# pdeljanov/Symphonia

Hardware: NVIDIA H100
Metric: decoded audio-seconds/sec (44.1kHz stereo) (higher is better)
Workload: dtype f32

## Files before the change

symphonia_b200/csrc/mp3_kernel.cu:

```cuda
#include <cuda_runtime.h>

#include <cstdint>
#include <cstdlib>

#include "../../include/symgpu.h"
#include "mp3_kernel.h"
#include "tables.h"

namespace symgpu {

struct Mp3Const {
    float imdct_win[4][36];
    float half_cos12[6][6];
    float dct_iv_scale[18];
    float sdct18_scale[9];
    float sdct9_d[7];
    float lee16[16], lee8[8], lee4[4], lee2[2], lee1;
    float is_mpeg1[7][2];
    float is_mpeg2[2][32][2];
    float cs[8], ca[8];
    uint8_t pre_emphasis[24];
    uint8_t mixed_switch[12];
    uint8_t n_edges[9][3];
};
__constant__ Mp3Const c_mp3;

cudaError_t mp3_upload_const(const Mp3Tables& t, cudaStream_t stream) {
    static Mp3Const h;
    memcpy(h.imdct_win, t.imdct_win, sizeof h.imdct_win);
    memcpy(h.half_cos12, t.half_cos12, sizeof h.half_cos12);
    memcpy(h.dct_iv_scale, t.dct_iv_scale, sizeof h.dct_iv_scale);
    memcpy(h.sdct18_scale, t.sdct18_scale, sizeof h.sdct18_scale);
    memcpy(h.sdct9_d, t.sdct9_d, sizeof h.sdct9_d);
    memcpy(h.lee16, t.lee16, sizeof h.lee16);
    memcpy(h.lee8, t.lee8, sizeof h.lee8);
    memcpy(h.lee4, t.lee4, sizeof h.lee4);
    memcpy(h.lee2, t.lee2, sizeof h.lee2);
    h.lee1 = t.lee1;
    memcpy(h.is_mpeg1, t.is_mpeg1, sizeof h.is_mpeg1);
    memcpy(h.is_mpeg2, t.is_mpeg2, sizeof h.is_mpeg2);
    memcpy(h.cs, t.cs, sizeof h.cs);
    memcpy(h.ca, t.ca, sizeof h.ca);
    memcpy(h.pre_emphasis, t.pre_emphasis, sizeof h.pre_emphasis);
    memset(h.mixed_switch, 0, sizeof h.mixed_switch);
    memcpy(h.mixed_switch, t.mixed_switch, 9);
    memcpy(h.n_edges, t.n_edges, sizeof h.n_edges);
    cudaError_t e = cudaMemcpyToSymbolAsync(c_mp3, &h, sizeof h, 0, cudaMemcpyHostToDevice, stream);
    if (e != cudaSuccess) return e;
    return cudaStreamSynchronize(stream);
}

namespace {

constexpr int kPitch = 33;
constexpr float kFrac1Sqrt2 = 0.707106781186547524400844362104849039f;

struct WarpScratch {
    symgpu_mp3_gc gc[2];
    float scale[2][40];
    float2 sratio[40];
    uint8_t smode[40];
    uint8_t nz[40];
    int next_region;
    Mp3StreamState* st_out;
};

__device__ __forceinline__ int kind_of(const symgpu_mp3_gc& g) {
    if (g.block_type != SYMGPU_MP3_SHORT) return kKindLong;
    return (g.flags & SYMGPU_MP3_F_MIXED) ? kKindMixed : kKindShort;
}

__device__ __forceinline__ void sdct9(const float (&x)[9], float (&y)[9]) {
    const float a01 = x[3] + x[5], a02 = x[3] - x[5], a03 = x[6] + x[2], a04 = x[6] - x[2];
    const float a05 = x[1] + x[7], a06 = x[1] - x[7], a07 = x[8] + x[0], a08 = x[8] - x[0];
    const float a09 = x[4] + a05, a10 = a01 + a03, a11 = a10 + a07, a12 = a03 - a07;
    const float a13 = a01 - a07, a14 = a01 - a03, a15 = a02 - a04, a16 = a15 + a08;
    const float a17 = a04 + a08, a18 = a02 - a08, a19 = a02 + a04, a20 = 2.0f * x[4] - a05;
    const float m1 = c_mp3.sdct9_d[0] * a06, m2 = c_mp3.sdct9_d[1] * a12, m3 = c_mp3.sdct9_d[2] * a13;
    const float m4 = c_mp3.sdct9_d[3] * a14, m5 = c_mp3.sdct9_d[0] * a16, m6 = c_mp3.sdct9_d[4] * a17;
    const float m7 = c_mp3.sdct9_d[5] * a18, m8 = c_mp3.sdct9_d[6] * a19;
    const float a21 = a20 + m2, a22 = a20 - m2, a23 = a20 + m3, a24 = m1 + m6, a25 = m1 - m6, a26 = m1 + m7;
    y[0] = a09 + a11;
    y[1] = m8 - a26;
    y[2] = m4 - a21;
    y[3] = m5;
    y[4] = a22 - m3;
    y[5] = a25 - m7;
    y[6] = a11 - 2.0f * a09;
    y[7] = a24 + m8;
    y[8] = a23 + m4;
}

__device__ __forceinline__ void dct_iv_18(const float (&x)[18], float (&y)[18]) {
    float s[18];
#pragma unroll
    for (int i = 0; i < 18; ++i) s[i] = c_mp3.dct_iv_scale[i] * x[i];
    float even[9], odd[9], ye[9], yo[9];
#pragma unroll
    for (int i = 0; i < 9; ++i) even[i] = s[i] + s[17 - i];
    sdct9(even, ye);
#pragma unroll
    for (int i = 0; i < 9; ++i) odd[i] = c_mp3.sdct18_scale[i] * (s[i] - s[17 - i]);
    sdct9(odd, yo);
#pragma unroll
    for (int j = 1; j < 9; ++j) yo[j] = yo[j] - yo[j - 1];
#pragma unroll
    for (int j = 0; j < 9; ++j) {
        y[2 * j] = ye[j];
        y[2 * j + 1] = yo[j];
    }
    y[0] = y[0] * 0.5f;
#pragma unroll
    for (int i = 1; i < 18; ++i) y[i] = (y[i] * 0.5f) - y[i - 1];
}

__device__ __forceinline__ void imdct36(const float (&x)[18], const float* __restrict__ win,
                                        float (&first)[18], float (&second)[18]) {
// ... 20 lines not shown
        for (int i = 0; i < 3; ++i) {
            const float yl = (x[w] * c_mp3.half_cos12[i][0]) + (x[3 + w] * c_mp3.half_cos12[i][1]) +
                             (x[6 + w] * c_mp3.half_cos12[i][2]) + (x[9 + w] * c_mp3.half_cos12[i][3]) +
                             (x[12 + w] * c_mp3.half_cos12[i][4]) + (x[15 + w] * c_mp3.half_cos12[i][5]);
            const float yr = (x[w] * c_mp3.half_cos12[i + 3][0]) + (x[3 + w] * c_mp3.half_cos12[i + 3][1]) +
                             (x[6 + w] * c_mp3.half_cos12[i + 3][2]) + (x[9 + w] * c_mp3.half_cos12[i + 3][3]) +
                             (x[12 + w] * c_mp3.half_cos12[i + 3][4]) + (x[15 + w] * c_mp3.half_cos12[i + 3][5]);
            tmp[6 + 6 * w + 2 - i] += -yl * win[2 - i];
            tmp[6 + 6 * w + i + 3] += yl * win[i + 3];
            tmp[6 + 6 * w + i + 6] += yr * win[i + 6];
            tmp[6 + 6 * w + 11 - i] += yr * win[11 - i];
        }
    }
#pragma unroll
    for (int i = 0; i < 18; ++i) {
        first[i] = tmp[i];
        second[i] = tmp[i + 18];
    }
}

template <int N> struct LeeCoef;
template <> struct LeeCoef<16> { static __device__ __forceinline__ float at(int i) { return c_mp3.lee16[i]; } };
template <> struct LeeCoef<8> { static __device__ __forceinline__ float at(int i) { return c_mp3.lee8[i]; } };
template <> struct LeeCoef<4> { static __device__ __forceinline__ float at(int i) { return c_mp3.lee4[i]; } };
template <> struct LeeCoef<2> { static __device__ __forceinline__ float at(int i) { return c_mp3.lee2[i]; } };

template <int N>
__device__ __forceinline__ void lee_dct(const float (&x)[N], float (&y)[N]) {
    if constexpr (N == 2) {
        y[0] = x[0] + x[1];
        y[1] = (x[0] - x[1]) * c_mp3.lee1;
    } else {
        constexpr int H = N / 2;
        float lo[H], hi[H], lo_t[H], hi_t[H];
#pragma unroll
        for (int i = 0; i < H; ++i) {
            lo[i] = x[i] + x[N - 1 - i];
            hi[i] = (x[i] - x[N - 1 - i]) * LeeCoef<H>::at(i);
        }
        lee_dct<H>(lo, lo_t);
        lee_dct<H>(hi, hi_t);
#pragma unroll
        for (int i = 0; i < H - 1; ++i) {
            y[2 * i] = lo_t[i];
            y[2 * i + 1] = hi_t[i] + hi_t[i + 1];
        }
        y[N - 2] = lo_t[H - 1];
        y[N - 1] = hi_t[H - 1];
    }
}

__device__ __forceinline__ float finv(float v, int sb, int t) { return ((sb & t) & 1) ? -v : v; }

}

namespace {

__device__ __forceinline__ uint32_t smem_u32(const void* p) { return (uint32_t)__cvta_generic_to_shared(p); }
__device__ __forceinline__ void mbar_init(uint64_t* bar, uint32_t count) {
    asm volatile("mbarrier.init.shared::cta.b64 [%0], %1;" ::"r"(smem_u32(bar)), "r"(count) : "memory");
}
__device__ __forceinline__ void mbar_expect_tx(uint64_t* bar, uint32_t bytes) {
    asm volatile("mbarrier.arrive.expect_tx.shared::cta.b64 _, [%0], %1;" ::"r"(smem_u32(bar)), "r"(bytes) : "memory");
}
__device__ __forceinline__ void mbar_wait(uint64_t* bar, uint32_t parity) {
    asm volatile(
        "{\n"
        ".reg .pred p;\n"
        "WAIT_%=:\n"
        "mbarrier.try_wait.parity.shared::cta.b64 p, [%0], %1;\n"
        "@p bra DONE_%=;\n"
        "bra WAIT_%=;\n"
        "DONE_%=:\n"
        "}\n" ::"r"(smem_u32(bar)),
        "r"(parity)
        : "memory");
}
__device__ __forceinline__ void tma_bulk_g2s(void* dst_smem, const void* src_gmem, uint32_t bytes, uint64_t* bar) {
    asm volatile("cp.async.bulk.shared::cluster.global.mbarrier::complete_tx::bytes [%0], [%1], %2, [%3];" ::"r"(
                     smem_u32(dst_smem)),
                 "l"(src_gmem), "r"(bytes), "r"(smem_u32(bar))
                 : "memory");
}

__device__ __forceinline__ float2 lds64(uint32_t addr) {
    float2 v;
    asm volatile("ld.shared.v2.f32 {%0, %1}, [%2];" : "=f"(v.x), "=f"(v.y) : "r"(addr));
    return v;
}


__device__ __forceinline__ float2 pk_mul(float2 a, float s) { return make_float2(__fmul_rn(a.x, s), __fmul_rn(a.y, s)); }
__device__ __forceinline__ float2 pk_add(float2 a, float2 b) { return make_float2(__fadd_rn(a.x, b.x), __fadd_rn(a.y, b.y)); }

template <bool TWO_JUMPS = false>
__device__ __forceinline__ void window_phase(const float* xt, int row0, int begin, int end, int lane,
                                             const float* __restrict__ synth_d, float* __restrict__ pcm, int slot_seq0,
                                             int slots_per_frame, bool stereo) {
    const int col_lo = lane < 16 ? 16 + lane : (lane == 16 ? 32 : 48 - lane);
    const int col_hi = lane <= 16 ? 16 - lane : lane - 16;
    float dlo[8], dhi[8];
#pragma unroll
    for (int j = 0; j < 8; ++j) {
        const float a0 = __ldg(synth_d + 64 * j + lane);
        dlo[j] = lane > 16 ? -a0 : a0;
        dhi[j] = -__ldg(synth_d + 64 * j + 32 + lane);
    }
    if (begin >= end) return;
    constexpr uint32_t kRowBytes = kPitch * 8;
    uint32_t a_lo = smem_u32(xt) + (uint32_t)((row0 + begin - 15) * kPitch + col_lo) * 8u;
    uint32_t a_hi = smem_u32(xt) + (uint32_t)((row0 + begin - 15) * kPitch + col_hi) * 8u;
    float2 wl[16], wh[16];
#pragma unroll
    for (int m = 0; m < 15; ++m) {
        wl[(m + 1) & 15] = lds64(a_lo + m * kRowBytes);
        wh[(m + 1) & 15] = lds64(a_hi + m * kRowBytes);
    }
    a_lo += 15 * kRowBytes;
    a_hi += 15 * kRowBytes;
    const int off1 = stereo ? 1152 : 0;
    const int frame_jump = SYMGPU_MP3_FRAME_FLOATS - slots_per_frame * 32;
    for (int base = begin; base < end; base += 16) {
        const int seq = slot_seq0 + base;
        const int frame = seq / slots_per_frame, sif = seq - frame * slots_per_frame;
        float* out0 = pcm + (size_t)frame * SYMGPU_MP3_FRAME_FLOATS + sif * 32 + lane;
        float* out1 = out0 + frame_jump;
        const int kj = slots_per_frame - sif;
        const int cnt = end - base;
#pragma unroll
        for (int u = 0; u < 16; ++u) {
            if (u < cnt) {
                wl[u] = lds64(a_lo + u * kRowBytes);
                wh[u] = lds64(a_hi + u * kRowBytes);
                float2 acc = make_float2(0.0f, 0.0f);
#pragma unroll
                for (int j = 0; j < 8; ++j) {
                    acc = pk_add(pk_mul(wl[(u - 2 * j) & 15], dlo[j]), acc);
                    acc = pk_add(pk_mul(wh[(u - 2 * j - 1) & 15], dhi[j]), acc);
                }
                float* o = (u < kj ? out0 : out1) + u * 32;
                if (TWO_JUMPS && u >= kj + slots_per_frame) o += frame_jump;
                o[off1] = acc.y;
                o[0] = acc.x;
            }
        }
        a_lo += 16 * kRowBytes;
        a_hi += 16 * kRowBytes;
    }
}

template <int T, int NW>
struct Mp3Smem {
    static constexpr int kRows = 18 * kMp3GroupRegions;
    float xt[kRows * kPitch * 2];
    alignas(16) float spec[NW][2 * 576];
    alignas(16) symgpu_mp3_gc units[NW][2];
    WarpScratch ws[NW];
    alignas(16) Mp3StreamState carry;
    alignas(16) Mp3Tile seg_stage[2][kMp3GroupTiles];
    uint32_t gen_stage[2][kMp3GroupTiles];
    int nseg_stage[2];
    alignas(8) uint64_t bar;
    bool is_last;
};

}

template <int T, int NW, bool MULTI>
__global__ void __launch_bounds__(NW * 32, NW <= 8 ? 2 : 1) mp3_synth_kernel(Mp3Args a) {
    static_assert(NW >= T, "one warp per granule job (a tile with a halo holds NW - 2 granules)");
    extern __shared__ __align__(16) unsigned char smem_raw[];
    using Smem = Mp3Smem<T, NW>;
    Smem& sm = *reinterpret_cast<Smem*>(smem_raw);
    float* xt = sm.xt;

    const int lane = threadIdx.x & 31;
    const int warp = threadIdx.x >> 5;
    const Mp3Tables* __restrict__ tab = a.tab;
    const int n_tiles = a.n_tiles;

    auto issue_prefetch = [&](int ti, int parity) {
        int nseg = 0, jobs = 0;
        for (;;) {
            const Mp3Tile t = a.tiles[ti + nseg];
            sm.seg_stage[parity][nseg] = t;
            sm.gen_stage[parity][nseg] = a.gen[t.stream];
            jobs += t.n_granules + ((t.flags & (kTileLoadState | kTileCarryIn)) ? 0 : 2);
            ++nseg;
            if (!MULTI || (t.flags & kTileGroupEnd) || nseg == kMp3GroupTiles) break;
        }
        sm.nseg_stage[parity] = nseg;
        mbar_expect_tx(&sm.bar, (uint32_t)jobs * (4608u + 128u));
        int slot0 = 0;
        for (int k = 0; k < nseg; ++k) {
            const Mp3Tile t = sm.seg_stage[parity][k];
            const int halo = (t.flags & (kTileLoadState | kTileCarryIn)) ? 0 : 2;
            const int cnt = t.n_granules + halo;
            if (t.gpf == 2) {
                const size_t src = (size_t)t.first_frame * 2 + t.first_gr - halo;
                tma_bulk_g2s(sm.spec[slot0], a.spectra + src * 1152, (uint32_t)cnt * 4608u, &sm.bar);
                tma_bulk_g2s(sm.units[slot0], a.units + src * 2, (uint32_t)cnt * 128u, &sm.bar);
            } else {
                for (int j = 0; j < cnt; ++j) {
                    const size_t src = (size_t)((int)t.first_frame + t.first_gr - halo + j) * 2;
                    tma_bulk_g2s(sm.spec[slot0 + j], a.spectra + src * 1152, 4608u, &sm.bar);
                    tma_bulk_g2s(sm.units[slot0 + j], a.units + src * 2, 128u, &sm.bar);
                }
            }
            slot0 += cnt;
        }
    };

    if (threadIdx.x == 0) {
        mbar_init(&sm.bar, 1);
        asm volatile("fence.mbarrier_init.release.cluster;" ::: "memory");
    }
    __syncthreads();
    const int t_begin = (int)a.cta_first[blockIdx.x], t_end = (int)a.cta_first[blockIdx.x + 1];
    if (threadIdx.x == 0 && t_begin < t_end) issue_prefetch(t_begin, 0);

    WarpScratch& ws = sm.ws[warp];
    int it = 0;
    for (int ti = t_begin; ti < t_end; ++it) {
        const int par = it & 1;
        mbar_wait(&sm.bar, (uint32_t)par);
        const int nseg = MULTI ? sm.nseg_stage[par] : 1;
        Mp3Tile tile = sm.seg_stage[par][0];
        int seg = -1, job0 = 0, reg0 = 0;
        {
            int jobs = 0, regions = 0;
            for (int k = 0; k < nseg; ++k) {
                const Mp3Tile t = sm.seg_stage[par][k];
                const int cnt = t.n_granules + ((t.flags & (kTileLoadState | kTileCarryIn)) ? 0 : 2);
                if (seg < 0 && warp < jobs + cnt) {
                    seg = k;
                    job0 = jobs;
                    reg0 = regions;
                    tile = t;
                }
                jobs += cnt;
                regions += t.n_granules + 1;
            }
        }
        const int n = tile.n_granules;
        const int n_ch = tile.n_ch;
        const bool load_state = tile.flags & (kTileLoadState | kTileCarryIn);
        const bool store_state = tile.flags & (kTileStoreState | kTileCarryOut);
        const uint32_t gen = sm.gen_stage[par][seg < 0 ? 0 : seg];
        const Mp3StreamState* st_in = (tile.flags & kTileCarryIn) ? &sm.carry : a.states + (size_t)tile.stream * 2 + (gen & 1);
        Mp3StreamState* st_out = (tile.flags & kTileCarryOut) ? &sm.carry : a.states + (size_t)tile.stream * 2 + ((gen + 1) & 1);
        const int j0 = load_state ? 2 : 0;

        const int g = warp - job0 + j0;
        const bool active = seg >= 0;
        if (lane == 0) {
            ws.next_region = (active && g + 1 < n + 2) ? reg0 + g : -1;
            ws.st_out = (active && g + 1 >= n + 2 && store_state) ? st_out : nullptr;
        }
        float sec[2][18];
        if (active) {
            const symgpu_mp3_gc& g0 = sm.units[warp][0];
            const symgpu_mp3_gc& g1 = sm.units[warp][1];
            const float* S = sm.spec[warp];
            if (lane < 10) reinterpret_cast<uint32_t*>(ws.smode)[lane] = 0;
            if (lane >= 16 && lane < 26) reinterpret_cast<uint32_t*>(ws.nz)[lane - 16] = 0;
            const int sr = g0.sample_rate_idx;
            const int kind0 = kind_of(g0), kind1 = (n_ch == 2) ? kind_of(g1) : kind0;
            const bool ms = (n_ch == 2) && (g0.flags & SYMGPU_MP3_F_MID_SIDE);
            const bool is = (n_ch == 2) && (g0.flags & SYMGPU_MP3_F_INTENSITY);
            int rz0 = g0.rzero, rz1 = (n_ch == 2) ? g1.rzero : 0;

            for (int ch = 0; ch < n_ch; ++ch) {
                const symgpu_mp3_gc& gg = sm.units[warp][ch];
                const int kind = ch ? kind1 : kind0;
                const int n_iv = c_mp3.n_edges[sr][kind] - 1;
                const int gain = (int)gg.global_gain - 210;
                const int shift = (gg.flags & SYMGPU_MP3_F_SCALEFAC_SCALE) ? 2 : 1;
                const int sw = c_mp3.mixed_switch[sr];
                for (int idx = lane; idx < 40; idx += 32) {
                    float s = 1.0f;
                    if (idx < n_iv) {
                        int e = 0;
                        bool scaled = true;
                        const bool long_part = (kind == kKindLong) || (kind == kKindMixed && idx < sw - 1);
                        if (long_part) {
                            const int pre = (gg.flags & SYMGPU_MP3_F_PREFLAG) ? c_mp3.pre_emphasis[idx] : 0;
                            const int b = ((gg.scalefacs[idx] + pre) << shift) & 0xff;
                            e = gain - b;
                        } else if (kind == kKindMixed && idx == sw - 1) {
                            scaled = false;
                        } else {
                            const int j = (kind == kKindMixed) ? idx - sw : idx;
                            const int b = (gg.scalefacs[idx] << shift) & 0xff;
                            e = gain - 8 * (int)gg.subblock_gain[j % 3] - b;
                        }
                        if (scaled) s = __ldg(&tab->pow2q[e - kPow2qMin]);
                    }
                    ws.scale[ch][idx] = s;
                }
            }
            __syncwarp();

            float x[2][18];
            uint32_t ivq[5] = {0u, 0u, 0u, 0u, 0u};
            const int rz_joint = max(rz0, rz1);
            const int rze[2] = {(ms || is) ? rz_joint : rz0, (ms || is) ? rz_joint : rz1};
            int rzr[2] = {rze[0], rze[1]};
#pragma unroll
            for (int ch = 0; ch < 2; ++ch) {
                if (ch >= n_ch) {
#pragma unroll
                    for (int i = 0; i < 18; ++i) x[ch][i] = 0.0f;
// ... 66 lines not shown
                        first_is0 = first_is1 = first_is2 = hb + 1;
                    } else {
                        const int sw = (kind1 == kKindMixed) ? c_mp3.mixed_switch[sr] : 0;
                        const int n_quads = (n_e - sw - 1) / 3;
                        int hq0 = -1, hq1 = -1, hq2 = -1;
                        for (int q = 0; q < n_quads; ++q) {
                            const unsigned bits = (unsigned)(nzmask >> (sw + 3 * q)) & 7u;
                            if (bits & 1u) hq0 = q;
                            if (bits & 2u) hq1 = q;
                            if (bits & 4u) hq2 = q;
                        }
                        const int qstop = min(hq0, min(hq1, hq2));
                        const int qlo = max(qstop, 0);
                        is_lo = sw + 3 * qlo;
                        first_is0 = sw + 3 * (hq0 + 1);
                        first_is1 = sw + 3 * (hq1 + 1) + 1;
                        first_is2 = sw + 3 * (hq2 + 1) + 2;
                        if (qstop < 0 && kind1 == kKindMixed) {
                            const unsigned long long lmask = nzmask & ((1ull << sw) - 1ull);
                            const int hb = lmask ? 63 - __clzll((long long)lmask) : -1;
                            if (hb < sw - 1) is_lo = hb + 1;
                        }
                    }
                    for (int iv = lane; iv < n_iv; iv += 32) {
                        uint8_t mode = mode_hi;
                        if (iv >= is_lo) {
                            bool coded;
                            if (kind1 == kKindLong) {
                                coded = true;
                            } else {
                                const int sw = (kind1 == kKindMixed) ? c_mp3.mixed_switch[sr] : 0;
                                if (iv < sw) coded = true;
                                else {
                                    const int w = (iv - sw) % 3;
                                    coded = iv >= (w == 0 ? first_is0 : w == 1 ? first_is1 : first_is2);
                                }
                            }
                            if (coded) {
                                const int k = (kind1 == kKindLong) ? (iv == 21 ? 20 : iv) : (iv < 36 ? iv : iv - 3);
                                const int pos = g1.scalefacs[k];
                                if (pos < inv_pos) {
                                    mode = 2;
                                    ws.sratio[iv] = __ldg(reinterpret_cast<const float2*>(rt[pos]));
                                }
                            }
                        }
                        ws.smode[iv] = mode;
                    }
                    __syncwarp();
#pragma unroll
                    for (int i = 0; i < 18; ++i) {
                        const int iv = (ivq[i >> 2] >> (8 * (i & 3))) & 0xff;
                        const int mode = ws.smode[iv];
                        const float l = x[0][i], r = x[1][i];
                        if (mode == 2) {
                            const float2 ratio = ws.sratio[iv];
                            x[0][i] = ratio.x * l;
                            x[1][i] = ratio.y * l;
                        } else if (mode == 1) {
                            x[0][i] = (l + r) * kFrac1Sqrt2;
                            x[1][i] = (l - r) * kFrac1Sqrt2;
                        }
                    }
                } else {
#pragma unroll
                    for (int i = 0; i < 18; ++i) {
                        const float l = x[0][i], r = x[1][i];
                        x[0][i] = (l + r) * kFrac1Sqrt2;
                        x[1][i] = (l - r) * kFrac1Sqrt2;
                    }
                }
            }

            int rzh[2];
#pragma unroll
            for (int ch = 0; ch < 2; ++ch) {
                const int kind = ch ? kind1 : kind0;
                rzh[ch] = rzr[ch];
                if (ch >= n_ch || kind == kKindShort) continue;
                const int sb_limit = (kind == kKindMixed) ? 2 : 32;
                const int rz = 18 * min(min(sb_limit, rzr[ch] / 18 + 2), 32);
                rzh[ch] = rz;
                float nb_lo[8], nb_up[8];
#pragma unroll
                for (int i = 0; i < 8; ++i) {
                    nb_lo[i] = __shfl_up_sync(0xffffffffu, x[ch][17 - i], 1);
                    nb_up[i] = __shfl_down_sync(0xffffffffu, x[ch][i], 1);
                }
                const bool do_bottom = lane >= 1 && 18 * lane < rz;
                const bool do_top = lane < 31 && 18 * (lane + 1) < rz;
#pragma unroll
                for (int i = 0; i < 8; ++i) {
                    const float up = x[ch][i], lo = x[ch][17 - i];
                    if (do_bottom) x[ch][i] = up * c_mp3.cs[i] + nb_lo[i] * c_mp3.ca[i];
                    if (do_top) x[ch][17 - i] = lo * c_mp3.cs[i] - nb_up[i] * c_mp3.ca[i];
                }
            }

            float* X = xt + (size_t)(18 * (reg0 + g - 1)) * kPitch * 2;
#pragma unroll
            for (int ch = 0; ch < 2; ++ch) {
                float first[18];
                if (ch < n_ch) {
                    const symgpu_mp3_gc& gg = sm.units[warp][ch];
                    const int kind = ch ? kind1 : kind0;
                    const int rz = rzh[ch];
                    const int sb_limit = (rz + 17) / 18;
                    const int sb_split = (kind == kKindShort) ? 0 : (kind == kKindMixed) ? 2 : 32;
                    const int long_end = min(sb_split, sb_limit);
                    if (lane < long_end) {
                        const int wsel = gg.block_type == SYMGPU_MP3_START ? 1 : gg.block_type == SYMGPU_MP3_END ? 3 : 0;
                        imdct36(x[ch], c_mp3.imdct_win[wsel], first, sec[ch]);
                    } else if (lane < sb_limit) {
                        imdct12x3(x[ch], first, sec[ch]);
                    } else {
#pragma unroll
                        for (int i = 0; i < 18; ++i) {
                            first[i] = -0.0f;
                            sec[ch][i] = 0.0f;
                        }
                    }
                } else {
#pragma unroll
                    for (int i = 0; i < 18; ++i) {
                        first[i] = 0.0f;
                        sec[ch][i] = 0.0f;
                    }
                }
                if (g == 2 && load_state) {
#pragma unroll
                    for (int t = 0; t < 18; ++t) first[t] = first[t] + st_in->overlap[ch][lane][t];
                }
                if (g >= 1) {
#pragma unroll
                    for (int t = 0; t < 18; ++t) X[(t * kPitch + lane) * 2 + ch] = finv(first[t], lane, t);
                }
            }
        }
        __syncthreads();
        if (threadIdx.x == NW * 32 - 32 && ti + nseg < t_end) {
            asm volatile("fence.proxy.async.shared::cta;" ::: "memory");
            issue_prefetch(ti + nseg, (it + 1) & 1);
        }
        {
            const int next_region = ws.next_region;
            Mp3StreamState* so = ws.st_out;
            if (next_region >= 0) {
                float* Xn = xt + (size_t)(18 * next_region) * kPitch * 2;
#pragma unroll
                for (int ch = 0; ch < 2; ++ch)
#pragma unroll
                    for (int t = 0; t < 18; ++t) {
                        float* p = Xn + (t * kPitch + lane) * 2 + ch;
                        *p = *p + finv(sec[ch][t], lane, t);
                    }
            } else if (so) {
#pragma unroll
                for (int ch = 0; ch < 2; ++ch)
#pragma unroll
                    for (int t = 0; t < 18; ++t) so->overlap[ch][lane][t] = sec[ch][t];
            }
        }
        {
            int regions = 0;
            for (int k = 0; k < nseg; ++k) {
                const Mp3Tile t = sm.seg_stage[par][k];
                if (t.flags & (kTileLoadState | kTileCarryIn)) {
                    const uint32_t gk = sm.gen_stage[par][k];
                    const Mp3StreamState* st = (t.flags & kTileCarryIn) ? &sm.carry : a.states + (size_t)t.stream * 2 + (gk & 1);
                    for (int idx = threadIdx.x; idx < 15 * kPitch; idx += NW * 32) {
                        const int srow = idx / kPitch, col = idx - srow * kPitch;
                        float2 v = make_float2(0.0f, 0.0f);
                        if (col < 32) v = st->dhist[srow][col];
                        *reinterpret_cast<float2*>(xt + (size_t)((18 * regions + 3 + srow) * kPitch + col) * 2) = v;
                    }
                }
                regions += t.n_granules + 1;
            }
        }
        __syncthreads();

        {
            int total_rows = 0;
            for (int k = 0; k < nseg; ++k) {
                const Mp3Tile t = sm.seg_stage[par][k];
                total_rows += 18 * t.n_granules + ((t.flags & (kTileLoadState | kTileCarryIn)) ? 0 : 15);
            }
            const int chn = lane >> 4;
            for (int base = warp * 16; base < total_rows; base += NW * 16) {
                int r = base + (lane & 15);
                if (r < total_rows) {
                    int regions = 0, row = 0;
                    for (int k = 0; k < nseg; ++k) {
                        const Mp3Tile t = sm.seg_stage[par][k];
                        const int lead = (t.flags & (kTileLoadState | kTileCarryIn)) ? 0 : 15;
                        const int cnt = 18 * t.n_granules + lead;
                        if (r < cnt) {
                            row = 18 * regions + 18 - lead + r;
                            break;
                        }
                        r -= cnt;
                        regions += t.n_granules + 1;
                    }
                    float* rowp = xt + (size_t)row * kPitch * 2 + chn;
                    float v[32], y[32];
#pragma unroll
                    for (int i = 0; i < 32; ++i) v[i] = rowp[2 * i];
                    lee_dct<32>(v, y);
#pragma unroll
                    for (int i = 0; i < 32; ++i) rowp[2 * i] = y[i];
                    rowp[64] = 0.0f;
                }
            }
        }
        __syncthreads();

        {
            int total_slots = 0;
            for (int k = 0; k < nseg; ++k) total_slots += 18 * sm.seg_stage[par][k].n_granules;
            const int per = (total_slots + NW - 1) / NW;
            const int my_begin = warp * per, my_end = min(total_slots, my_begin + per);
            int regions = 0, first = 0;
            for (int k = 0; k < nseg; ++k) {
                const Mp3Tile t = sm.seg_stage[par][k];
                const int cnt = 18 * t.n_granules;
                const int b = max(my_begin, first) - first, e = min(my_end, first + cnt) - first;
                if (b < e) {
                    const int shift = t.gpf == 2 ? 1 : 0;
                    const int gseq = ((int)t.first_frame << shift) + t.first_gr;
                    window_phase(xt, 18 * (regions + 1), b, e, lane, tab->synth_d, a.pcm, gseq * 18, 18 << shift, t.n_ch == 2);
                }
                first += cnt;
                regions += t.n_granules + 1;
            }
        }
        __syncthreads();
        {
            int regions = 0;
            for (int k = 0; k < nseg; ++k) {
                const Mp3Tile t = sm.seg_stage[par][k];
                if (t.flags & (kTileStoreState | kTileCarryOut)) {
                    const uint32_t gk = sm.gen_stage[par][k];
                    Mp3StreamState* st = (t.flags & kTileCarryOut) ? &sm.carry : a.states + (size_t)t.stream * 2 + ((gk + 1) & 1);
                    const float* last = xt + (size_t)(18 * (regions + t.n_granules + 1) - 15) * kPitch * 2;
                    for (int idx = threadIdx.x; idx < 15 * 32; idx += NW * 32) {
                        const int srow = idx >> 5, col = idx & 31;
                        st->dhist[srow][col] = *reinterpret_cast<const float2*>(last + (size_t)(srow * kPitch + col) * 2);
                    }
                }
                regions += t.n_granules + 1;
            }
        }
        ti += nseg;
        __syncthreads();
    }

    __syncthreads();
    if (threadIdx.x == 0) {
        __threadfence();
        sm.is_last = atomicAdd(a.done, 1u) == gridDim.x - 1;
    }
    __syncthreads();
    if (sm.is_last) {
        for (int i = threadIdx.x; i < n_tiles; i += NW * 32)
            if (a.tiles[i].flags & kTileStoreState) a.gen[a.tiles[i].stream] += 1;
        if (threadIdx.x == 0) *a.done = 0;
    }
}

namespace {
constexpr int kMpa12Slots = 288;
struct Mpa12Smem {
    float xt[(18 + kMpa12Slots) * kPitch * 2];
    bool is_last;
};
}

template <int NW>
__global__ void __launch_bounds__(NW * 32, 1) mpa12_synth_kernel(Mpa12Args a) {
    extern __shared__ __align__(16) unsigned char smem_raw[];
    Mpa12Smem& sm = *reinterpret_cast<Mpa12Smem*>(smem_raw);
    float* xt = sm.xt;
    const int lane = threadIdx.x & 31, warp = threadIdx.x >> 5;
    const int n_slots = a.n_slots;
    const Mp3Tables* __restrict__ tab = a.tab;
    const int t_begin = (int)a.cta_first[blockIdx.x], t_end = (int)a.cta_first[blockIdx.x + 1];
    for (int ti = t_begin; ti < t_end; ++ti) {
        const Mp3Tile tile = a.tiles[ti];
        const int n = tile.n_granules;
        const int total = n * n_slots;
        const bool from_state = tile.flags & kTileLoadState, carried = tile.flags & kTileCarryIn;
        const uint32_t gen = a.gen[tile.stream];
        const Mp3StreamState* st_in = a.states + (size_t)tile.stream * 2 + (gen & 1);
        Mp3StreamState* st_out = a.states + (size_t)tile.stream * 2 + ((gen + 1) & 1);
        const float* in = a.subbands + (size_t)tile.first_frame * 64 * n_slots;
        if (from_state) {
            for (int idx = threadIdx.x; idx < 15 * kPitch; idx += NW * 32) {
                const int srow = idx / kPitch, col = idx - srow * kPitch;
                float2 v = make_float2(0.0f, 0.0f);
                if (col < 32) v = st_in->dhist[srow][col];
                *reinterpret_cast<float2*>(xt + (size_t)((3 + srow) * kPitch + col) * 2) = v;
            }
        } else if (!carried) {
            for (int idx = threadIdx.x; idx < 15 * 64; idx += NW * 32) {
                const int j = idx >> 6, sb = (idx >> 1) & 31, ch = idx & 1;
                const int gslot = (int)tile.first_frame * n_slots - 15 + j;
                const int f = gslot / n_slots, s = gslot - f * n_slots;
// ... 89 lines not shown
    }
    if (a.n_ctas <= 0) return cudaErrorInvalidConfiguration;
    mpa12_synth_kernel<kMp3Warps><<<a.n_ctas, kMp3Warps * 32, smem, stream>>>(a);
    return cudaGetLastError();
}

int mp3_tile_granules() {
    static int t = 0;
    if (!t) {
        t = kMp3TileGranules;
        if (const char* env = getenv("SYMGPU_MP3_T")) {
            const int v = atoi(env);
            if (v >= 4 && v <= kMp3TileGranules) t = v;
        }
    }
    return t;
}
int mp3_cta_warps() { return kMp3Warps; }
int mp3_halo_tile_granules() { return kMp3Warps - 2 < mp3_tile_granules() ? kMp3Warps - 2 : mp3_tile_granules(); }

int mp3_grid_size(cudaError_t* err) {
    constexpr size_t smem = sizeof(Mp3Smem<kMp3TileGranules, kMp3Warps>);
    static int grid_for_device[64] = {0};
    int dev = 0;
    cudaError_t e = cudaGetDevice(&dev);
    if (e == cudaSuccess && !grid_for_device[dev & 63]) {
        int n_sm = 0, per_sm = 0;
        e = cudaFuncSetAttribute(mp3_synth_kernel<kMp3TileGranules, kMp3Warps, false>, cudaFuncAttributeMaxDynamicSharedMemorySize, (int)smem);
        if (e == cudaSuccess)
            e = cudaFuncSetAttribute(mp3_synth_kernel<kMp3TileGranules, kMp3Warps, true>, cudaFuncAttributeMaxDynamicSharedMemorySize, (int)smem);
        if (e == cudaSuccess) e = cudaDeviceGetAttribute(&n_sm, cudaDevAttrMultiProcessorCount, dev);
        if (e == cudaSuccess)
            e = cudaOccupancyMaxActiveBlocksPerMultiprocessor(&per_sm, mp3_synth_kernel<kMp3TileGranules, kMp3Warps, true>, kMp3Warps * 32, smem);
        if (e == cudaSuccess) grid_for_device[dev & 63] = n_sm * (per_sm > 0 ? per_sm : 1);
    }
    if (err) *err = e;
    return e == cudaSuccess ? grid_for_device[dev & 63] : 0;
}

cudaError_t mp3_launch(const Mp3Args& a, cudaStream_t stream) {
    constexpr size_t smem = sizeof(Mp3Smem<kMp3TileGranules, kMp3Warps>);
    cudaError_t e = cudaSuccess;
    const int max_grid = mp3_grid_size(&e);
    if (e != cudaSuccess) return e;
    if (a.n_ctas <= 0 || a.n_ctas > max_grid) return cudaErrorInvalidConfiguration;
    if (a.multi_tile_groups)
        mp3_synth_kernel<kMp3TileGranules, kMp3Warps, true><<<a.n_ctas, kMp3Warps * 32, smem, stream>>>(a);
    else
        mp3_synth_kernel<kMp3TileGranules, kMp3Warps, false><<<a.n_ctas, kMp3Warps * 32, smem, stream>>>(a);
    return cudaGetLastError();
}

}
```

Before: 1.296 million.

## Replace block barrier for IMDCT overlap-add with pairwise named barriers

Each warp now parks its second IMDCT half in its spectrum scratch. It signals only the next warp through a named barrier (bar.arrive/bar.sync), and the receiving warp does the overlap-add. This removes one full __syncthreads, and the dhist state load moves ahead of the IMDCT phase. The carry state is double-buffered by parity and the synthesis window table is staged into shared memory. Optional clock probes are added under a compile flag. The change risks ordering hazards, since spec scratch is reused and named barrier IDs must not collide with other barriers.

New measurement: 1.367 million, median of 6. 1.05x the previous value.

```diff
diff --git a/symphonia_b200/csrc/mp3_kernel.cu b/symphonia_b200/csrc/mp3_kernel.cu
--- a/symphonia_b200/csrc/mp3_kernel.cu
+++ b/symphonia_b200/csrc/mp3_kernel.cu
@@ -61,8 +61,6 @@
     float2 sratio[40];
     uint8_t smode[40];
     uint8_t nz[40];
-    int next_region;
-    Mp3StreamState* st_out;
 };
 
 __device__ __forceinline__ int kind_of(const symgpu_mp3_gc& g) {
@@ -230,7 +228,7 @@
 __device__ __forceinline__ float2 pk_mul(float2 a, float s) { return make_float2(__fmul_rn(a.x, s), __fmul_rn(a.y, s)); }
 __device__ __forceinline__ float2 pk_add(float2 a, float2 b) { return make_float2(__fadd_rn(a.x, b.x), __fadd_rn(a.y, b.y)); }
 
-template <bool TWO_JUMPS = false>
+template <bool TWO_JUMPS = false, bool SMEM_D = false>
 __device__ __forceinline__ void window_phase(const float* xt, int row0, int begin, int end, int lane,
                                              const float* __restrict__ synth_d, float* __restrict__ pcm, int slot_seq0,
                                              int slots_per_frame, bool stereo) {
@@ -239,9 +237,9 @@
     float dlo[8], dhi[8];
 #pragma unroll
     for (int j = 0; j < 8; ++j) {
-        const float a0 = __ldg(synth_d + 64 * j + lane);
+        const float a0 = SMEM_D ? synth_d[64 * j + lane] : __ldg(synth_d + 64 * j + lane);
         dlo[j] = lane > 16 ? -a0 : a0;
-        dhi[j] = -__ldg(synth_d + 64 * j + 32 + lane);
+        dhi[j] = -(SMEM_D ? synth_d[64 * j + 32 + lane] : __ldg(synth_d + 64 * j + 32 + lane));
     }
     if (begin >= end) return;
     constexpr uint32_t kRowBytes = kPitch * 8;
@@ -293,15 +291,45 @@
     alignas(16) float spec[NW][2 * 576];
     alignas(16) symgpu_mp3_gc units[NW][2];
     WarpScratch ws[NW];
-    alignas(16) Mp3StreamState carry;
+    alignas(16) Mp3StreamState carry[2];
     alignas(16) Mp3Tile seg_stage[2][kMp3GroupTiles];
     uint32_t gen_stage[2][kMp3GroupTiles];
     int nseg_stage[2];
     alignas(8) uint64_t bar;
+    float synth_d[512];
     bool is_last;
 };
 
 }
+
+#ifdef SYMGPU_MP3_PHASE_CLOCKS
+constexpr int kClkMaxCtas = 256, kClkMaxGroups = 32, kClkWords = 96, kClkBarriers = 4;
+constexpr int kClkTop = 0, kClkTma = 1, kClkArrive = 2, kClkRelease = kClkArrive + 16 * kClkBarriers;
+constexpr int kClkNsTop = kClkRelease + kClkBarriers, kClkNsEnd = kClkNsTop + 1, kClkGranules = kClkNsEnd + 1;
+__device__ unsigned long long g_mp3_clk[kClkMaxCtas][kClkMaxGroups][kClkWords];
+__device__ __forceinline__ unsigned long long global_ns() {
+    unsigned long long t;
+    asm volatile("mov.u64 %0, %%globaltimer;" : "=l"(t)::"memory");
+    return t;
+}
+__device__ __forceinline__ unsigned long long sm_clock() {
+    unsigned long long t;
+    asm volatile("mov.u64 %0, %%clock64;" : "=l"(t)::"memory");
+    return t;
+}
+#define MP3_CLK_AT(i) \
+    if (clk && threadIdx.x == 0) clk[i] = sm_clock()
+#define MP3_CLK_NS(i) \
+    if (clk && threadIdx.x == 0) clk[i] = global_ns()
+#define MP3_CLK_ARRIVE(b) \
+    if (clk && lane == 0) clk[kClkArrive + 16 * (b) + warp] = sm_clock()
+#define MP3_CLK_RELEASE(b) MP3_CLK_AT(kClkRelease + (b))
+#else
+#define MP3_CLK_AT(i) ((void)0)
+#define MP3_CLK_NS(i) ((void)0)
+#define MP3_CLK_ARRIVE(b) ((void)0)
+#define MP3_CLK_RELEASE(b) ((void)0)
+#endif
 
 template <int T, int NW, bool MULTI>
 __global__ void __launch_bounds__(NW * 32, NW <= 8 ? 2 : 1) mp3_synth_kernel(Mp3Args a) {
@@ -352,6 +380,7 @@
         mbar_init(&sm.bar, 1);
         asm volatile("fence.mbarrier_init.release.cluster;" ::: "memory");
     }
+    for (int i = threadIdx.x; i < 512; i += NW * 32) sm.synth_d[i] = __ldg(tab->synth_d + i);
     __syncthreads();
     const int t_begin = (int)a.cta_first[blockIdx.x], t_end = (int)a.cta_first[blockIdx.x + 1];
     if (threadIdx.x == 0 && t_begin < t_end) issue_prefetch(t_begin, 0);
@@ -359,8 +388,14 @@
     WarpScratch& ws = sm.ws[warp];
     int it = 0;
     for (int ti = t_begin; ti < t_end; ++it) {
+#ifdef SYMGPU_MP3_PHASE_CLOCKS
+        unsigned long long* clk = (blockIdx.x < kClkMaxCtas && it < kClkMaxGroups) ? g_mp3_clk[blockIdx.x][it] : nullptr;
+        MP3_CLK_NS(kClkNsTop);
+        MP3_CLK_AT(kClkTop);
+#endif
         const int par = it & 1;
         mbar_wait(&sm.bar, (uint32_t)par);
+        MP3_CLK_AT(kClkTma);
         const int nseg = MULTI ? sm.nseg_stage[par] : 1;
         Mp3Tile tile = sm.seg_stage[par][0];
         int seg = -1, job0 = 0, reg0 = 0;
@@ -381,20 +416,36 @@
         }
         const int n = tile.n_granules;
         const int n_ch = tile.n_ch;
+#ifdef SYMGPU_MP3_PHASE_CLOCKS
+        if (clk && threadIdx.x == 0) clk[kClkGranules] = (unsigned long long)n | ((unsigned long long)tile.flags << 16);
+#endif
         const bool load_state = tile.flags & (kTileLoadState | kTileCarryIn);
         const bool store_state = tile.flags & (kTileStoreState | kTileCarryOut);
         const uint32_t gen = sm.gen_stage[par][seg < 0 ? 0 : seg];
-        const Mp3StreamState* st_in = (tile.flags & kTileCarryIn) ? &sm.carry : a.states + (size_t)tile.stream * 2 + (gen & 1);
-        Mp3StreamState* st_out = (tile.flags & kTileCarryOut) ? &sm.carry : a.states + (size_t)tile.stream * 2 + ((gen + 1) & 1);
+        const Mp3StreamState* st_in = (tile.flags & kTileCarryIn) ? &sm.carry[par] : a.states + (size_t)tile.stream * 2 + (gen & 1);
+        Mp3StreamState* st_out = (tile.flags & kTileCarryOut) ? &sm.carry[par ^ 1] : a.states + (size_t)tile.stream * 2 + ((gen + 1) & 1);
         const int j0 = load_state ? 2 : 0;
+
+        {
+            int regions = 0;
+            for (int k = 0; k < nseg; ++k) {
+                const Mp3Tile t = sm.seg_stage[par][k];
+                if (t.flags & (kTileLoadState | kTileCarryIn)) {
+                    const uint32_t gk = sm.gen_stage[par][k];
+                    const Mp3StreamState* st = (t.flags & kTileCarryIn) ? &sm.carry[par] : a.states + (size_t)t.stream * 2 + (gk & 1);
+                    for (int idx = threadIdx.x; idx < 15 * kPitch; idx += NW * 32) {
+                        const int srow = idx / kPitch, col = idx - srow * kPitch;
+                        float2 v = make_float2(0.0f, 0.0f);
+                        if (col < 32) v = st->dhist[srow][col];
+                        *reinterpret_cast<float2*>(xt + (size_t)((18 * regions + 3 + srow) * kPitch + col) * 2) = v;
+                    }
+                }
+                regions += t.n_granules + 1;
+            }
+        }
 
         const int g = warp - job0 + j0;
         const bool active = seg >= 0;
-        if (lane == 0) {
-            ws.next_region = (active && g + 1 < n + 2) ? reg0 + g : -1;
-            ws.st_out = (active && g + 1 >= n + 2 && store_state) ? st_out : nullptr;
-        }
-        float sec[2][18];
         if (active) {
             const symgpu_mp3_gc& g0 = sm.units[warp][0];
             const symgpu_mp3_gc& g1 = sm.units[warp][1];
@@ -612,10 +663,12 @@
                 }
             }
 
+            const bool has_next = g + 1 < n + 2;
+            const bool has_prev = g > j0;
             float* X = xt + (size_t)(18 * (reg0 + g - 1)) * kPitch * 2;
 #pragma unroll
             for (int ch = 0; ch < 2; ++ch) {
-                float first[18];
+                float first[18], second[18];
                 if (ch < n_ch) {
                     const symgpu_mp3_gc& gg = sm.units[warp][ch];
                     const int kind = ch ? kind1 : kind0;
@@ -625,22 +678,30 @@
                     const int long_end = min(sb_split, sb_limit);
                     if (lane < long_end) {
                         const int wsel = gg.block_type == SYMGPU_MP3_START ? 1 : gg.block_type == SYMGPU_MP3_END ? 3 : 0;
-                        imdct36(x[ch], c_mp3.imdct_win[wsel], first, sec[ch]);
+                        imdct36(x[ch], c_mp3.imdct_win[wsel], first, second);
                     } else if (lane < sb_limit) {
-                        imdct12x3(x[ch], first, sec[ch]);
+                        imdct12x3(x[ch], first, second);
                     } else {
 #pragma unroll
                         for (int i = 0; i < 18; ++i) {
                             first[i] = -0.0f;
-                            sec[ch][i] = 0.0f;
+                            second[i] = 0.0f;
                         }
                     }
                 } else {
 #pragma unroll
                     for (int i = 0; i < 18; ++i) {
                         first[i] = 0.0f;
-                        sec[ch][i] = 0.0f;
-                    }
+                        second[i] = 0.0f;
+                    }
+                }
+                if (has_next) {
+                    float* park = sm.spec[warp] + ch * 576 + lane;
+#pragma unroll
+                    for (int t = 0; t < 18; ++t) park[32 * t] = second[t];
+                } else if (store_state) {
+#pragma unroll
+                    for (int t = 0; t < 18; ++t) st_out->overlap[ch][lane][t] = second[t];
                 }
                 if (g == 2 && load_state) {
 #pragma unroll
@@ -651,49 +712,26 @@
                     for (int t = 0; t < 18; ++t) X[(t * kPitch + lane) * 2 + ch] = finv(first[t], lane, t);
                 }
             }
-        }
+            if (has_next) asm volatile("bar.arrive %0, 64;" ::"r"(warp + 1) : "memory");
+            if (has_prev) {
+                asm volatile("bar.sync %0, 64;" ::"r"(warp) : "memory");
+                const float* park = sm.spec[warp - 1] + lane;
+#pragma unroll
+                for (int ch = 0; ch < 2; ++ch)
+#pragma unroll
+                    for (int t = 0; t < 18; ++t) {
+                        float* p = X + (t * kPitch + lane) * 2 + ch;
+                        *p = *p + finv(park[ch * 576 + 32 * t], lane, t);
+                    }
+            }
+        }
+        MP3_CLK_ARRIVE(0);
         __syncthreads();
+        MP3_CLK_RELEASE(0);
         if (threadIdx.x == NW * 32 - 32 && ti + nseg < t_end) {
             asm volatile("fence.proxy.async.shared::cta;" ::: "memory");
             issue_prefetch(ti + nseg, (it + 1) & 1);
         }
-        {
-            const int next_region = ws.next_region;
-            Mp3StreamState* so = ws.st_out;
-            if (next_region >= 0) {
-                float* Xn = xt + (size_t)(18 * next_region) * kPitch * 2;
-#pragma unroll
-                for (int ch = 0; ch < 2; ++ch)
-#pragma unroll
-                    for (int t = 0; t < 18; ++t) {
-                        float* p = Xn + (t * kPitch + lane) * 2 + ch;
-                        *p = *p + finv(sec[ch][t], lane, t);
-                    }
-            } else if (so) {
-#pragma unroll
-                for (int ch = 0; ch < 2; ++ch)
-#pragma unroll
-                    for (int t = 0; t < 18; ++t) so->overlap[ch][lane][t] = sec[ch][t];
-            }
-        }
-        {
-            int regions = 0;
-            for (int k = 0; k < nseg; ++k) {
-                const Mp3Tile t = sm.seg_stage[par][k];
-                if (t.flags & (kTileLoadState | kTileCarryIn)) {
-                    const uint32_t gk = sm.gen_stage[par][k];
-                    const Mp3StreamState* st = (t.flags & kTileCarryIn) ? &sm.carry : a.states + (size_t)t.stream * 2 + (gk & 1);
-                    for (int idx = threadIdx.x; idx < 15 * kPitch; idx += NW * 32) {
-                        const int srow = idx / kPitch, col = idx - srow * kPitch;
-                        float2 v = make_float2(0.0f, 0.0f);
-                        if (col < 32) v = st->dhist[srow][col];
-                        *reinterpret_cast<float2*>(xt + (size_t)((18 * regions + 3 + srow) * kPitch + col) * 2) = v;
-                    }
-                }
-                regions += t.n_granules + 1;
-            }
-        }
-        __syncthreads();
 
         {
             int total_rows = 0;
@@ -728,7 +766,9 @@
                 }
             }
         }
+        MP3_CLK_ARRIVE(1);
         __syncthreads();
+        MP3_CLK_RELEASE(1);
 
         {
             int total_slots = 0;
@@ -743,20 +783,22 @@
                 if (b < e) {
                     const int shift = t.gpf == 2 ? 1 : 0;
                     const int gseq = ((int)t.first_frame << shift) + t.first_gr;
-                    window_phase(xt, 18 * (regions + 1), b, e, lane, tab->synth_d, a.pcm, gseq * 18, 18 << shift, t.n_ch == 2);
+                    window_phase<false, true>(xt, 18 * (regions + 1), b, e, lane, sm.synth_d, a.pcm, gseq * 18, 18 << shift, t.n_ch == 2);
                 }
                 first += cnt;
                 regions += t.n_granules + 1;
             }
         }
+        MP3_CLK_ARRIVE(2);
         __syncthreads();
+        MP3_CLK_RELEASE(2);
         {
             int regions = 0;
             for (int k = 0; k < nseg; ++k) {
                 const Mp3Tile t = sm.seg_stage[par][k];
                 if (t.flags & (kTileStoreState | kTileCarryOut)) {
                     const uint32_t gk = sm.gen_stage[par][k];
-                    Mp3StreamState* st = (t.flags & kTileCarryOut) ? &sm.carry : a.states + (size_t)t.stream * 2 + ((gk + 1) & 1);
+                    Mp3StreamState* st = (t.flags & kTileCarryOut) ? &sm.carry[par ^ 1] : a.states + (size_t)t.stream * 2 + ((gk + 1) & 1);
                     const float* last = xt + (size_t)(18 * (regions + t.n_granules + 1) - 15) * kPitch * 2;
                     for (int idx = threadIdx.x; idx < 15 * 32; idx += NW * 32) {
                         const int srow = idx >> 5, col = idx & 31;
@@ -767,7 +809,10 @@
             }
         }
         ti += nseg;
+        MP3_CLK_ARRIVE(3);
         __syncthreads();
+        MP3_CLK_RELEASE(3);
+        MP3_CLK_NS(kClkNsEnd);
     }
 
     __syncthreads();
@@ -963,3 +1008,14 @@
 }
 
 }
+
+#ifdef SYMGPU_MP3_PHASE_CLOCKS
+extern "C" size_t symgpu_debug_mp3_phase_clocks(void* out, size_t cap) {
+    const size_t bytes = sizeof(symgpu::g_mp3_clk);
+    if (cap < bytes) return 0;
+    if (cudaDeviceSynchronize() != cudaSuccess || cudaMemcpyFromSymbol(out, symgpu::g_mp3_clk, bytes) != cudaSuccess) return 0;
+    void* dev = nullptr;
+    if (cudaGetSymbolAddress(&dev, symgpu::g_mp3_clk) != cudaSuccess || cudaMemset(dev, 0, bytes) != cudaSuccess) return 0;
+    return cudaDeviceSynchronize() == cudaSuccess ? bytes : 0;
+}
+#endif
```

## Park IMDCT overlap halves in smem and fold overlap-add into DCT pass

Applied to the files above, without the earlier changes.

Each warp now writes its second IMDCT half into a swizzled per-warp shared-memory park buffer instead of keeping it in registers. The overlap-add with the next granule is done while loading rows for the 32-point Lee DCT, which removes one __syncthreads phase and the separate read-modify-write pass over the time buffer. The dhist state load moves before the IMDCT phase, the next-tile prefetch is issued later, and branchy stereo processing becomes selects. Optional clock64 phase instrumentation is added behind a compile flag. This reduces register pressure and barriers at the cost of extra shared-memory traffic and index arithmetic in the DCT loop.

Result: faster. 1.298 million before, 1.410 million after, median of 6 (+8.6%).

```diff
diff --git a/symphonia_b200/csrc/mp3_kernel.cu b/symphonia_b200/csrc/mp3_kernel.cu
--- a/symphonia_b200/csrc/mp3_kernel.cu
+++ b/symphonia_b200/csrc/mp3_kernel.cu
@@ -50,6 +50,20 @@
     return cudaStreamSynchronize(stream);
 }
 
+#ifdef SYMGPU_MP3_PHASE_CLOCKS
+constexpr int kClkCtas = 160, kClkIters = 16, kClkWarps = 16, kClkStamps = 12;
+__device__ unsigned long long g_mp3_clk[kClkCtas][kClkIters][kClkWarps][kClkStamps];
+#define MP3_CLK(k)                                                                                      \
+    do {                                                                                                \
+        if (lane == 0 && blockIdx.x < kClkCtas && it < kClkIters && warp < kClkWarps)                   \
+            g_mp3_clk[blockIdx.x][it][warp][k] = clock64();                                             \
+    } while (0)
+#else
+#define MP3_CLK(k) \
+    do {           \
+    } while (0)
+#endif
+
 namespace {
 
 constexpr int kPitch = 33;
@@ -61,7 +75,6 @@
     float2 sratio[40];
     uint8_t smode[40];
     uint8_t nz[40];
-    int next_region;
     Mp3StreamState* st_out;
 };
 
@@ -189,6 +202,10 @@
 
 __device__ __forceinline__ float finv(float v, int sb, int t) { return ((sb & t) & 1) ? -v : v; }
 
+__device__ __forceinline__ int park_row(int ch, int t) { return (ch * 18 + t) * 32; }
+__device__ __forceinline__ int park_quad(int q, int t) { return ((q + t) & 7) << 2; }
+__device__ __forceinline__ int park_index(int ch, int t, int sb) { return park_row(ch, t) + park_quad(sb >> 2, t) + (sb & 3); }
+
 }
 
 namespace {
@@ -360,7 +377,9 @@
     int it = 0;
     for (int ti = t_begin; ti < t_end; ++it) {
         const int par = it & 1;
+        MP3_CLK(11);
         mbar_wait(&sm.bar, (uint32_t)par);
+        MP3_CLK(0);
         const int nseg = MULTI ? sm.nseg_stage[par] : 1;
         Mp3Tile tile = sm.seg_stage[par][0];
         int seg = -1, job0 = 0, reg0 = 0;
@@ -388,13 +407,28 @@
         Mp3StreamState* st_out = (tile.flags & kTileCarryOut) ? &sm.carry : a.states + (size_t)tile.stream * 2 + ((gen + 1) & 1);
         const int j0 = load_state ? 2 : 0;
 
+        {
+            int regions = 0;
+            for (int k = 0; k < nseg; ++k) {
+                const Mp3Tile t = sm.seg_stage[par][k];
+                if (t.flags & (kTileLoadState | kTileCarryIn)) {
+                    const uint32_t gk = sm.gen_stage[par][k];
+                    const Mp3StreamState* st = (t.flags & kTileCarryIn) ? &sm.carry : a.states + (size_t)t.stream * 2 + (gk & 1);
+                    for (int idx = threadIdx.x; idx < 15 * kPitch; idx += NW * 32) {
+                        const int srow = idx / kPitch, col = idx - srow * kPitch;
+                        float2 v = make_float2(0.0f, 0.0f);
+                        if (col < 32) v = st->dhist[srow][col];
+                        *reinterpret_cast<float2*>(xt + (size_t)((18 * regions + 3 + srow) * kPitch + col) * 2) = v;
+                    }
+                }
+                regions += t.n_granules + 1;
+            }
+        }
+
         const int g = warp - job0 + j0;
         const bool active = seg >= 0;
-        if (lane == 0) {
-            ws.next_region = (active && g + 1 < n + 2) ? reg0 + g : -1;
-            ws.st_out = (active && g + 1 >= n + 2 && store_state) ? st_out : nullptr;
-        }
-        float sec[2][18];
+        if (lane == 0) ws.st_out = (active && g + 1 >= n + 2 && store_state) ? st_out : nullptr;
+        float* park = sm.spec[warp];
         if (active) {
             const symgpu_mp3_gc& g0 = sm.units[warp][0];
             const symgpu_mp3_gc& g1 = sm.units[warp][1];
@@ -567,15 +601,12 @@
                     for (int i = 0; i < 18; ++i) {
                         const int iv = (ivq[i >> 2] >> (8 * (i & 3))) & 0xff;
                         const int mode = ws.smode[iv];
+                        const float2 ratio = ws.sratio[iv];
                         const float l = x[0][i], r = x[1][i];
-                        if (mode == 2) {
-                            const float2 ratio = ws.sratio[iv];
-                            x[0][i] = ratio.x * l;
-                            x[1][i] = ratio.y * l;
-                        } else if (mode == 1) {
-                            x[0][i] = (l + r) * kFrac1Sqrt2;
-                            x[1][i] = (l - r) * kFrac1Sqrt2;
-                        }
+                        const float i0 = ratio.x * l, i1 = ratio.y * l;
+                        const float m0 = (l + r) * kFrac1Sqrt2, m1 = (l - r) * kFrac1Sqrt2;
+                        x[0][i] = mode == 2 ? i0 : mode == 1 ? m0 : l;
+                        x[1][i] = mode == 2 ? i1 : mode == 1 ? m1 : r;
                     }
                 } else {
 #pragma unroll
@@ -615,7 +646,7 @@
             float* X = xt + (size_t)(18 * (reg0 + g - 1)) * kPitch * 2;
 #pragma unroll
             for (int ch = 0; ch < 2; ++ch) {
-                float first[18];
+                float first[18], sec[18];
                 if (ch < n_ch) {
                     const symgpu_mp3_gc& gg = sm.units[warp][ch];
                     const int kind = ch ? kind1 : kind0;
@@ -625,23 +656,25 @@
                     const int long_end = min(sb_split, sb_limit);
                     if (lane < long_end) {
                         const int wsel = gg.block_type == SYMGPU_MP3_START ? 1 : gg.block_type == SYMGPU_MP3_END ? 3 : 0;
-                        imdct36(x[ch], c_mp3.imdct_win[wsel], first, sec[ch]);
+                        imdct36(x[ch], c_mp3.imdct_win[wsel], first, sec);
                     } else if (lane < sb_limit) {
-                        imdct12x3(x[ch], first, sec[ch]);
+                        imdct12x3(x[ch], first, sec);
                     } else {
 #pragma unroll
                         for (int i = 0; i < 18; ++i) {
                             first[i] = -0.0f;
-                            sec[ch][i] = 0.0f;
+                            sec[i] = 0.0f;
                         }
                     }
                 } else {
 #pragma unroll
                     for (int i = 0; i < 18; ++i) {
                         first[i] = 0.0f;
-                        sec[ch][i] = 0.0f;
-                    }
-                }
+                        sec[i] = 0.0f;
+                    }
+                }
+#pragma unroll
+                for (int t = 0; t < 18; ++t) park[park_index(ch, t, lane)] = sec[t];
                 if (g == 2 && load_state) {
 #pragma unroll
                     for (int t = 0; t < 18; ++t) first[t] = first[t] + st_in->overlap[ch][lane][t];
@@ -652,48 +685,17 @@
                 }
             }
         }
+        MP3_CLK(1);
         __syncthreads();
-        if (threadIdx.x == NW * 32 - 32 && ti + nseg < t_end) {
-            asm volatile("fence.proxy.async.shared::cta;" ::: "memory");
-            issue_prefetch(ti + nseg, (it + 1) & 1);
-        }
-        {
-            const int next_region = ws.next_region;
-            Mp3StreamState* so = ws.st_out;
-            if (next_region >= 0) {
-                float* Xn = xt + (size_t)(18 * next_region) * kPitch * 2;
-#pragma unroll
-                for (int ch = 0; ch < 2; ++ch)
-#pragma unroll
-                    for (int t = 0; t < 18; ++t) {
-                        float* p = Xn + (t * kPitch + lane) * 2 + ch;
-                        *p = *p + finv(sec[ch][t], lane, t);
-                    }
-            } else if (so) {
-#pragma unroll
-                for (int ch = 0; ch < 2; ++ch)
-#pragma unroll
-                    for (int t = 0; t < 18; ++t) so->overlap[ch][lane][t] = sec[ch][t];
-            }
-        }
-        {
-            int regions = 0;
-            for (int k = 0; k < nseg; ++k) {
-                const Mp3Tile t = sm.seg_stage[par][k];
-                if (t.flags & (kTileLoadState | kTileCarryIn)) {
-                    const uint32_t gk = sm.gen_stage[par][k];
-                    const Mp3StreamState* st = (t.flags & kTileCarryIn) ? &sm.carry : a.states + (size_t)t.stream * 2 + (gk & 1);
-                    for (int idx = threadIdx.x; idx < 15 * kPitch; idx += NW * 32) {
-                        const int srow = idx / kPitch, col = idx - srow * kPitch;
-                        float2 v = make_float2(0.0f, 0.0f);
-                        if (col < 32) v = st->dhist[srow][col];
-                        *reinterpret_cast<float2*>(xt + (size_t)((18 * regions + 3 + srow) * kPitch + col) * 2) = v;
-                    }
-                }
-                regions += t.n_granules + 1;
-            }
-        }
-        __syncthreads();
+        MP3_CLK(2);
+        if (Mp3StreamState* so = ws.st_out) {
+#pragma unroll
+            for (int ch = 0; ch < 2; ++ch)
+#pragma unroll
+                for (int t = 0; t < 18; ++t) so->overlap[ch][lane][t] = park[park_index(ch, t, lane)];
+        }
+        MP3_CLK(3);
+        MP3_CLK(4);
 
         {
             int total_rows = 0;
@@ -705,22 +707,37 @@
             for (int base = warp * 16; base < total_rows; base += NW * 16) {
                 int r = base + (lane & 15);
                 if (r < total_rows) {
-                    int regions = 0, row = 0;
+                    int regions = 0, jobs = 0, row = 0, src = -1, tq = 0;
                     for (int k = 0; k < nseg; ++k) {
                         const Mp3Tile t = sm.seg_stage[par][k];
-                        const int lead = (t.flags & (kTileLoadState | kTileCarryIn)) ? 0 : 15;
+                        const bool has_state = t.flags & (kTileLoadState | kTileCarryIn);
+                        const int lead = has_state ? 0 : 15;
                         const int cnt = 18 * t.n_granules + lead;
                         if (r < cnt) {
-                            row = 18 * regions + 18 - lead + r;
+                            const int lr = 18 - lead + r, gj = lr / 18;
+                            row = 18 * regions + lr;
+                            tq = lr - 18 * gj;
+                            if (gj >= (has_state ? 2 : 0)) src = jobs + gj - (has_state ? 2 : 0);
                             break;
                         }
                         r -= cnt;
                         regions += t.n_granules + 1;
+                        jobs += t.n_granules + (has_state ? 0 : 2);
                     }
                     float* rowp = xt + (size_t)row * kPitch * 2 + chn;
+                    const float* sp = sm.spec[src < 0 ? 0 : src] + park_row(chn, tq);
                     float v[32], y[32];
 #pragma unroll
-                    for (int i = 0; i < 32; ++i) v[i] = rowp[2 * i];
+                    for (int q = 0; q < 8; ++q) {
+                        const float4 p = *reinterpret_cast<const float4*>(sp + park_quad(q, tq));
+                        const float pe[4] = {p.x, p.y, p.z, p.w};
+#pragma unroll
+                        for (int e = 0; e < 4; ++e) {
+                            const int i = 4 * q + e;
+                            const float sec = src >= 0 ? finv(pe[e], i, tq) : -0.0f;
+                            v[i] = rowp[2 * i] + sec;
+                        }
+                    }
                     lee_dct<32>(v, y);
 #pragma unroll
                     for (int i = 0; i < 32; ++i) rowp[2 * i] = y[i];
@@ -728,7 +745,13 @@
                 }
             }
         }
+        MP3_CLK(5);
         __syncthreads();
+        MP3_CLK(6);
+        if (threadIdx.x == NW * 32 - 32 && ti + nseg < t_end) {
+            asm volatile("fence.proxy.async.shared::cta;" ::: "memory");
+            issue_prefetch(ti + nseg, (it + 1) & 1);
+        }
 
         {
             int total_slots = 0;
@@ -749,7 +772,9 @@
                 regions += t.n_granules + 1;
             }
         }
+        MP3_CLK(7);
         __syncthreads();
+        MP3_CLK(8);
         {
             int regions = 0;
             for (int k = 0; k < nseg; ++k) {
@@ -767,7 +792,9 @@
             }
         }
         ti += nseg;
+        MP3_CLK(9);
         __syncthreads();
+        MP3_CLK(10);
     }
 
     __syncthreads();
@@ -963,3 +990,21 @@
 }
 
 }
+
+#ifdef SYMGPU_MP3_PHASE_CLOCKS
+extern "C" size_t symgpu_debug_mp3_phase_clocks(void* dst, size_t cap, int* dims) {
+    constexpr size_t bytes = sizeof(symgpu::g_mp3_clk);
+    if (dims) {
+        dims[0] = symgpu::kClkCtas;
+        dims[1] = symgpu::kClkIters;
+        dims[2] = symgpu::kClkWarps;
+        dims[3] = symgpu::kClkStamps;
+    }
+    if (!dst) return bytes;
+    if (cap < bytes || cudaDeviceSynchronize() != cudaSuccess) return 0;
+    if (cudaMemcpyFromSymbol(dst, symgpu::g_mp3_clk, bytes) != cudaSuccess) return 0;
+    void* p = nullptr;
+    if (cudaGetSymbolAddress(&p, symgpu::g_mp3_clk) != cudaSuccess || cudaMemset(p, 0, bytes) != cudaSuccess) return 0;
+    return cudaDeviceSynchronize() == cudaSuccess ? bytes : 0;
+}
+#endif
```
